# dpeerlab/segger

Hardware: AMD Instinct MI355X
Metric: edges scored/sec (tx->cell) fwd+bwd (higher is better)
Workload: dtype bf16; 1 GPU; C2: single Xenium-scale tile per GPU, 1000000 tx, 10000 nuclei, k=15 kNN (Ett=15000000, Etb=393796, Ep=2435646), training step fwd+bwd+Adam, attention dropout 0.2; parallelism=dp1

## Files before the change

### include/segger_amd.h

```cpp
#ifndef SEGGER_AMD_H
#define SEGGER_AMD_H

#include <stddef.h>
#include <stdint.h>

#ifdef __cplusplus
extern "C" {
#endif

#if defined(__GNUC__) || defined(__clang__)
#pragma GCC visibility push(default)
#endif

#define SEGGER_ABI_VERSION 30

enum segger_status {
  SEGGER_OK = 0,
  SEGGER_EINVAL = -1,
  SEGGER_EUNSUPPORTED = -2,
  SEGGER_EHIP = -3,
  SEGGER_EWORKSPACE = -4
};

enum segger_dtype { SEGGER_F32 = 0, SEGGER_BF16 = 1, SEGGER_F16 = 2 };

typedef void* segger_stream_t;

int segger_abi_version(void);
const char* segger_last_error(void);
// ... 381 lines not shown
                             float max_period, float* grad_w0, float* grad_b0, void* workspace, size_t workspace_bytes,
                             segger_stream_t stream);
int segger_posmlp_fwd(const float* pos, const int64_t* batch, const float* mins, const float* maxs, int64_t n, float eps,
                      float max_period, const void* w0, const float* b0, const void* w2, const float* b2, void* pe,
                      void* z1, float* pn, void* h1, void* pe_pre, int32_t gelu, int32_t dtype, segger_stream_t stream);
size_t segger_posmlp_bwd_workspace_bytes(int64_t n_rows);
int segger_posmlp_bwd(const void* g, int64_t ld_g, const void* z1, const float* pn, const void* w2_t, int64_t n_rows,
                      float max_period, int32_t dtype, float* grad_w0, float* grad_b0, float* grad_w2, float* grad_b2,
                      void* workspace, size_t workspace_bytes, segger_stream_t stream);
size_t segger_posmlp_bwd_pair_workspace_bytes(int64_t n_rows_a, int64_t n_rows_b);
int segger_posmlp_bwd_pair(const void* g_a, int64_t ld_ga, const void* z1_a, const float* pn_a, int64_t n_rows_a,
                           const void* g_b, int64_t ld_gb, const void* z1_b, const float* pn_b, int64_t n_rows_b,
                           const void* w2_t, float max_period, int32_t dtype, float* grad_w0, float* grad_b0,
                           float* grad_w2, float* grad_b2, void* workspace, size_t workspace_bytes,
                           segger_stream_t stream);
int segger_posmlp_wgrad(const void* dz1, int64_t ld_dz1, const float* pn, int64_t n_rows, float max_period,
                        int32_t dtype, float* grad_w0, float* grad_b0, void* workspace, size_t workspace_bytes,
                        segger_stream_t stream);
int segger_embed_gelu_fwd(const float* table, const int32_t* ids, const void* pe, int64_t ld_pe, int64_t n,
                          int32_t n_rows_table, int32_t D, void* out, int64_t ld_out, int32_t dtype,
                          segger_stream_t stream);
size_t segger_embed_gelu_bwd_workspace_bytes(int64_t n, int32_t n_rows_table, int32_t D);
int segger_embed_gelu_bwd(const void* gx0, int64_t ld_g, const float* table, const void* pe, int64_t ld_pe,
                          int64_t n, int32_t n_rows_table, int32_t D, void* gpe, int64_t ld_gpe, float* gtable,
                          const int64_t* gene_ptr, const int32_t* gene_rows, void* workspace, size_t workspace_bytes,
                          int32_t dtype, segger_stream_t stream);
typedef struct segger_front_join_args {
  const float* table; const int32_t* ids; int32_t n_rows_table; int32_t D; int32_t dtype; int32_t reserved_;
  const void* pe; int64_t ld_pe; int64_t n_tx, n_bd;
  const void* xb; int64_t ld_xb;
// ... 42 lines not shown
```

### segger_amd/_lib.py

```python
from __future__ import annotations

import ctypes as C
import os
from typing import Optional

import torch

_HERE = os.path.dirname(os.path.abspath(__file__))
LIB_PATH = os.environ.get("SEGGER_AMD_LIB") or os.path.join(_HERE, "libsegger_amd.so")
ABI_VERSION = 30

SEGGER_F32, SEGGER_BF16, SEGGER_F16 = 0, 1, 2
DTYPE_CODE = {torch.float32: SEGGER_F32, torch.bfloat16: SEGGER_BF16, torch.float16: SEGGER_F16}


class SeggerAmdError(RuntimeError):
    pass


c_i64p = C.c_void_p
vp = C.c_void_p


class Csr(C.Structure):
    _fields_ = [("indptr", vp), ("col", vp), ("eid", vp),
# ... 234 lines not shown
    "segger_gatv2_fwd_pair": (C.c_int, [vp, vp, vp]),
    "segger_gatv2_bwd_pair": (C.c_int, [vp, vp, vp]),
    "segger_pack_refresh": (C.c_int, [vp, C.c_int32, C.c_int32, vp]),
    "segger_dropout_bits_many": (C.c_int, [vp, C.c_int32, C.c_int32, C.c_float, vp, vp]),
    "segger_step_advance": (C.c_int, [vp, C.c_int64, vp, vp]),
    "segger_step_draws": (C.c_int, [C.POINTER(StepDrawsArgs), vp]),
    "segger_segment_minmax_ex": (C.c_int, [vp, vp, C.c_int64, C.c_int64, vp, vp, C.c_int32, vp]),
    "segger_triplet_partial_count": (C.c_int64, [C.c_int64]),
    "segger_loss_combine_partials_fwd": (C.c_int, [vp, vp, vp, vp, vp, C.c_int32, vp, vp]),
    "segger_posmlp_bwd_workspace_bytes": (C.c_size_t, [C.c_int64]),
    "segger_posmlp_bwd": (C.c_int, [vp, C.c_int64, vp, vp, vp, C.c_int64, C.c_float, C.c_int32, vp, vp, vp, vp, vp,
                                    C.c_size_t, vp]),
    "segger_posmlp_bwd_pair_workspace_bytes": (C.c_size_t, [C.c_int64, C.c_int64]),
    "segger_posmlp_bwd_pair": (C.c_int, [vp, C.c_int64, vp, vp, C.c_int64, vp, C.c_int64, vp, vp, C.c_int64, vp, C.c_float,
                                         C.c_int32, vp, vp, vp, vp, vp, C.c_size_t, vp]),
    "segger_linear_wgrad_dx_gate_supported": (C.c_int, [C.c_int32, C.c_int32, C.c_int32]),
    "segger_linear_wgrad_dx": (C.c_int, [vp, C.c_int64, vp, C.c_int64, vp, C.c_int64, C.c_int32, C.c_int32, C.c_int32, vp, vp,
                                         vp, C.c_int64, vp, C.c_int64, vp, C.c_size_t, vp]),
    "segger_posfreq": (C.c_int, [vp, vp, vp, vp, C.c_int64, C.c_int32, C.c_float, C.c_float, vp, C.c_int32, vp]),
    "segger_posenc_poly_supported": (C.c_int, [C.c_int32, C.c_int32]),
    "segger_posenc_poly_coef": (C.c_int, [vp, vp, C.c_int32, C.c_int32, C.c_float, vp, vp]),
    "segger_posenc_poly_fwd": (C.c_int, [vp, vp, vp, vp, C.c_int64, C.c_float, vp, C.c_int32, vp, vp, vp, vp]),
    "segger_posenc_poly_wgrad_workspace_bytes": (C.c_size_t, [C.c_int64, C.c_int32]),
    "segger_posenc_poly_wgrad": (C.c_int, [vp, C.c_int64, vp, C.c_int64, C.c_int32, C.c_int32, C.c_float, vp, vp, vp, C.c_size_t, vp]),
    "segger_embed_gelu_fwd": (C.c_int, [vp, vp, vp, C.c_int64, C.c_int64, C.c_int32, C.c_int32, vp, C.c_int64, C.c_int32, vp]),
    "segger_linear_fwd_f32_split_rowbias": (C.c_int, [vp, C.c_int64, vp, vp, C.c_int64, vp, vp, C.c_int64, C.c_int64, C.c_int32, C.c_int32, vp]),
    "segger_linear_fwd_f32_act": (C.c_int, [vp, C.c_int64, vp, vp, vp, C.c_int64, vp, C.c_int64, C.c_int32, C.c_int64, C.c_int32, C.c_int32, vp]),
    "segger_linear_fwd_f32_gate": (C.c_int, [vp, C.c_int64, vp, C.c_int32, vp, C.c_int64, C.c_int32, vp, C.c_int64, C.c_int64, C.c_int32, C.c_int32, vp]),
    "segger_f32_split_planes": (C.c_int, [vp, C.c_int32, C.c_int32, C.c_int32, vp, vp]),
    "segger_f32_split_planes_many": (C.c_int, [vp, C.c_int32, vp]),
# ... 97 lines not shown
```

### segger_amd/csrc/common.h

```cpp
#pragma once
#include <hip/hip_runtime.h>
#include <stdint.h>
#include <stdio.h>
#include <stdarg.h>
#include "../../include/segger_amd.h"

namespace segger {

void set_error(const char* fmt, ...);
int hip_fail(hipError_t e, const char* what);

#define SEGGER_REQUIRE(cond, ...)                 \
  do {                                            \
    if (!(cond)) {                                \
      ::segger::set_error(__VA_ARGS__);           \
      return SEGGER_EINVAL;                       \
    }                                             \
  } while (0)

#define SEGGER_HIP(call)                                        \
  do {                                                          \
    hipError_t _e = (call);                                     \
    if (_e != hipSuccess) return ::segger::hip_fail(_e, #call); \
  } while (0)
// ... 10 lines not shown
  static int cache[64] = {};
  int dev = 0;
  if (hipGetDevice(&dev) != hipSuccess || dev < 0) return 0;
  if (dev < 64 && cache[dev] > 0) return cache[dev];
  int n = 0;
  if (hipDeviceGetAttribute(&n, hipDeviceAttributeMultiprocessorCount, dev) != hipSuccess) n = 0;
  if (dev < 64 && n > 0) cache[dev] = n;
  return n;
}

int linear_f32_launch(const void* x, int64_t ldx, const void* w, const float* bias, void* y, int64_t ldy, int64_t n_rows,
                      int k_in, int m_out, hipStream_t stream, const float* rowbias = nullptr, const int32_t* rowidx = nullptr,
                      int64_t ld_rb = 0, const float* gate = nullptr, int64_t ld_gate = 0, int gate_kind = 0,
                      float* y_act = nullptr, int64_t ld_yact = 0, int act_kind = 0);
size_t wgrad_f32_workspace_bytes(int64_t n_rows, int m_out, int k_in);
bool wgrad_f32_split_shape_ok(int m, int k);
int64_t wgrad_f32_split_grid(int64_t n_rows, int m, int k);
int wgrad_f32_split_launch(const float* dy, int64_t ld_dy, const float* x, int64_t ld_x, int64_t n_rows, int m_out, int k_in,
                           float* partial, int64_t* n_slabs, hipStream_t stream);
int wgrad_f32_launch(const void* dy, int64_t ld_dy, const void* x, int64_t ld_x, int64_t n_rows, int m_out, int k_in,
                     float* partial, int64_t* n_slabs, hipStream_t stream);

struct ReduceSeg {
  const float* partial; int64_t n_slabs; int64_t width; int64_t split; float* out0; float* out1;
  float* scratch;
};
constexpr int kReduceGroups = 32;
bool defer_reduce(const ReduceSeg& seg, hipStream_t stream);

constexpr int kWave = 64;
// ... 170 lines not shown
```

### segger_amd/csrc/linear_wgrad.hip

```cpp
#include <cstdlib>
#include "common.h"

namespace segger {
namespace {

typedef __bf16   bf16x8 __attribute__((ext_vector_type(8)));
typedef _Float16 f16x8  __attribute__((ext_vector_type(8)));
typedef __bf16   bf16x2v __attribute__((ext_vector_type(2)));
typedef _Float16 f16x2v  __attribute__((ext_vector_type(2)));
typedef float    f32x16 __attribute__((ext_vector_type(16)));
typedef short    s16x4  __attribute__((ext_vector_type(4)));
typedef uint32_t u32x2  __attribute__((ext_vector_type(2)));
typedef uint32_t u32x4v __attribute__((ext_vector_type(4)));

constexpr int kStageRows = 16;

template <typename T> struct WgMfma;
template <> struct WgMfma<bf16_t> {
  static __device__ __forceinline__ f32x16 run(u32x4 a, u32x4 b, f32x16 c) {
    return __builtin_amdgcn_mfma_f32_32x32x16_bf16(__builtin_bit_cast(bf16x8, a), __builtin_bit_cast(bf16x8, b), c, 0, 0, 0);
  }
  static __device__ __forceinline__ f32x4 run16(u32x4 a, u32x4 b, f32x4 c) {
    return __builtin_amdgcn_mfma_f32_16x16x32_bf16(__builtin_bit_cast(bf16x8, a), __builtin_bit_cast(bf16x8, b), c, 0, 0, 0);
  }
// ... 338 lines not shown
  const void* z1;
  const float* pn;
  const void* w2t;
  int64_t n_rows, n_stages, stages_per_block;
  float* part2;
  float* part0;
  float log_max_period;
};
constexpr int kPbD = 64, kPbF = 256;
constexpr int kPbS = kPbD * 2 + 64;
constexpr int kPbTile = kStageRows * kPbS;
constexpr int kPbOffZ = kPbTile, kPbOffP = 2 * kPbTile;
constexpr int kPbBuf = 8 * 1024;
constexpr int kPbAhead = 6, kPbSlots = kPbAhead + 2;
constexpr int kPbWidth2 = kPbD * kPbD + kPbD, kPbWidth0 = kPbD * kPbF + kPbD;

__device__ __forceinline__ float sigmoid_fast(float z) {
  return __builtin_amdgcn_rcpf(1.0f + __builtin_amdgcn_exp2f(-1.4426950408889634f * z));
}

template <typename T>
__global__ __launch_bounds__(512, 2) void posmlp_bwd_kernel(PosBwdParams pa, PosBwdParams pb, int n_first) {
  const bool second = (int)blockIdx.x >= n_first;
  const PosBwdParams& p = second ? pb : pa;
  const int bid = second ? (int)blockIdx.x - n_first : (int)blockIdx.x;
  constexpr int D = kPbD, F = kPbF, S = kPbS, NW = 8, BUF = kPbBuf, NB = kPbSlots, TILE = kPbTile;
  __shared__ __attribute__((aligned(1024))) unsigned char lds[NB * BUF + 4 * TILE];
  unsigned char* tile_h = lds + NB * BUF;
  unsigned char* tile_d = tile_h + 2 * TILE;
  const int tid = threadIdx.x, lane = tid & 63;
  const int wave = __builtin_amdgcn_readfirstlane(tid >> 6);
  const T* __restrict__ gp = static_cast<const T*>(p.g);
  const T* __restrict__ zp = static_cast<const T*>(p.z1);

  const int64_t s_beg = (int64_t)bid * p.stages_per_block;
  int64_t s_end = s_beg + p.stages_per_block;
  if (s_end > p.n_stages) s_end = p.n_stages;
  const int n_local = (int)(s_end > s_beg ? s_end - s_beg : 0);
  const int64_t row_beg = s_beg * kStageRows;
  int64_t span_rows = p.n_rows > row_beg ? p.n_rows - row_beg : 0;
  if (span_rows > (int64_t)n_local * kStageRows) span_rows = (int64_t)n_local * kStageRows;
  i32x4 rs; int stage_bytes, voff;
// ... 20 lines not shown
  auto issue = [&](int local_stage) {
    lds_dma16(rs, lds_base + (uint32_t)((local_stage % NB) * BUF + wave * 1024), voff, local_stage * stage_bytes);
  };

  const int g4 = lane >> 4, i16 = lane & 15, tq = i16 >> 2, tp = i16 & 3;
  const int off_a = (8 * (g4 >> 1) + tq) * S + (16 * (g4 & 1) + 4 * tp) * 2;
  const int wm2 = wave & 1, wk2 = (wave >> 1) & 1;
  const int dq = lane >> 4, dj = lane & 15;
  const int r = lane & 31, h = lane >> 5;
  const bool lo_half = wave < 4;

  f32x16 acc2, acc0[2];
#pragma unroll
  for (int e = 0; e < 16; ++e) { acc2[e] = 0.f; acc0[0][e] = 0.f; acc0[1][e] = 0.f; }
  float db2 = 0.f, db0[2] = {0.f, 0.f};
  const float omega = expf(-p.log_max_period * (float)((32 * wave + r) % (F / 2)) / (float)(F / 2)) * 0.15915494309189535f;
  u32x4 wf[2] = {u32x4{0, 0, 0, 0}, u32x4{0, 0, 0, 0}};
  if (lo_half) {
    const T* wt = static_cast<const T*>(p.w2t);
#pragma unroll
    for (int ks = 0; ks < 2; ++ks)
      wf[ks] = *reinterpret_cast<const u32x4*>(wt + (16 * wave + dj) * D + 32 * ks + 8 * dq);
  }
  __builtin_amdgcn_s_waitcnt(0x0F70);
  asm volatile("" : "+v"(wf[0]), "+v"(wf[1]));

  auto consume = [&](int t) {
    const unsigned char* pb = lds + (t % NB) * BUF;
    const unsigned char* th = tile_h + (t & 1) * TILE;
    const unsigned char* td = tile_d + (t & 1) * TILE;
    if (lo_half) {
      const u32x2 lo = lds_read_tr(pb + off_a + wm2 * 64), hi = lds_read_tr(pb + off_a + wm2 * 64 + 4 * S);
      const u32x4 fa = u32x4{lo.x, lo.y, hi.x, hi.y};
      if (wk2 == 0) {
        db2 = WgMfma<T>::sum2(fa.x, db2); db2 = WgMfma<T>::sum2(fa.y, db2);
        db2 = WgMfma<T>::sum2(fa.z, db2); db2 = WgMfma<T>::sum2(fa.w, db2);
      }
      const u32x2 lo2 = lds_read_tr(th + off_a + wk2 * 64), hi2 = lds_read_tr(th + off_a + wk2 * 64 + 4 * S);
      acc2 = WgMfma<T>::run(fa, u32x4{lo2.x, lo2.y, hi2.x, hi2.y}, acc2);
    }
    u32x4 fd[2];
#pragma unroll
    for (int a = 0; a < 2; ++a) {
      const u32x2 lo = lds_read_tr(td + off_a + a * 64), hi = lds_read_tr(td + off_a + a * 64 + 4 * S);
      fd[a] = u32x4{lo.x, lo.y, hi.x, hi.y};
    }
    if (wave == 7) {
#pragma unroll
      for (int a = 0; a < 2; ++a) {
        float d = db0[a];
        d = WgMfma<T>::sum2(fd[a].x, d); d = WgMfma<T>::sum2(fd[a].y, d);
        d = WgMfma<T>::sum2(fd[a].z, d); d = WgMfma<T>::sum2(fd[a].w, d);
        db0[a] = d;
      }
    }
// ... 35 lines not shown
#pragma unroll
      for (int ks = 0; ks < 2; ++ks) {
        const u32x4 fy = *reinterpret_cast<const u32x4*>(base + dj * S + (32 * ks + 8 * dq) * 2);
        dacc = WgMfma<T>::run16(wf[ks], fy, dacc);
      }
      const u32x2 zv = *reinterpret_cast<const u32x2*>(base + kPbOffZ + dj * S + (16 * wave + 4 * dq) * 2);
      float z[4];
      Vec8<T>::unpack2(zv.x, z[0], z[1]);
      Vec8<T>::unpack2(zv.y, z[2], z[3]);
      float o[4] = {dacc.x, dacc.y, dacc.z, dacc.w};
#pragma unroll
      for (int e = 0; e < 4; ++e) {
        const float sg = sigmoid_fast(z[e]);
        o[e] *= sg * (1.0f + z[e] * (1.0f - sg));
      }
      *reinterpret_cast<u32x2*>(tile_d + (s & 1) * TILE + dj * S + (16 * wave + 4 * dq) * 2) =
          u32x2{Vec8<T>::pack(o[0], o[1]), Vec8<T>::pack(o[2], o[3])};
    }
    if (s > 0) consume(s - 1);
  }
  if (n_local > 0) {
    __builtin_amdgcn_s_waitcnt(0xC07F);
    __builtin_amdgcn_s_barrier();
    consume(n_local - 1);
  }
  __builtin_amdgcn_s_waitcnt(0x0F70);

  float* out2 = p.part2 + (int64_t)bid * kPbWidth2;
  float* out0 = p.part0 + (int64_t)bid * kPbWidth0;
#pragma unroll
  for (int e = 0; e < 16; ++e) {
    const int m = (e & 3) + 8 * (e >> 2) + 4 * h;
    if (lo_half) out2[(32 * wm2 + m) * D + 32 * wk2 + r] = acc2[e];
#pragma unroll
    for (int a = 0; a < 2; ++a) out0[(32 * a + m) * F + 32 * wave + r] = acc0[a][e];
  }
  if (lo_half && wk2 == 0) {
    const float d = db2 + __shfl_xor(db2, 32, 64);
    if (h == 0) out2[D * D + 32 * wm2 + r] = d;
  }
  if (wave == 7) {
#pragma unroll
    for (int a = 0; a < 2; ++a) {
      const float d = db0[a] + __shfl_xor(db0[a], 32, 64);
      if (h == 0) out0[D * F + 32 * a + r] = d;
    }
  }
}

constexpr int kRedGroups = 32;
__global__ __launch_bounds__(256) void wgrad_reduce1_kernel(const float* __restrict__ partial, int64_t n_slabs, int64_t width,
                                                           float* __restrict__ part2) {
  const int64_t e = (int64_t)blockIdx.x * 256 + threadIdx.x;
  if (e >= width) return;
  const int g = blockIdx.y;
  float s0 = 0.f, s1 = 0.f, s2 = 0.f, s3 = 0.f;
  int64_t s = g;
  for (; s + 3 * kRedGroups < n_slabs; s += 4 * kRedGroups) {
    s0 += partial[s * width + e];                    s1 += partial[(s + kRedGroups) * width + e];
    s2 += partial[(s + 2 * kRedGroups) * width + e]; s3 += partial[(s + 3 * kRedGroups) * width + e];
  }
  for (; s < n_slabs; s += kRedGroups) s0 += partial[s * width + e];
// ... 395 lines not shown

static int64_t posmlp_bwd_grid(int64_t n_rows) {
  const int64_t stages = (n_rows + kStageRows - 1) / kStageRows;
  const int64_t want = (stages + kMinStagesPerBlock - 1) / kMinStagesPerBlock;
  const int64_t cap = 2 * kNumCu;
  return want < cap ? (want < 1 ? 1 : want) : cap;
}

extern "C" size_t segger_posmlp_bwd_pair_workspace_bytes(int64_t n_rows_a, int64_t n_rows_b) {
  const int64_t grid = (n_rows_a > 0 ? posmlp_bwd_grid(n_rows_a) : 0) + (n_rows_b > 0 ? posmlp_bwd_grid(n_rows_b) : 0);
  if (grid == 0) return 16;
  return (size_t)(grid + kRedGroups) * (size_t)(kPbWidth2 + kPbWidth0) * sizeof(float);
}
extern "C" size_t segger_posmlp_bwd_workspace_bytes(int64_t n_rows) { return segger_posmlp_bwd_pair_workspace_bytes(n_rows, 0); }

extern "C" int segger_posmlp_bwd_pair(const void* g_a, int64_t ld_ga, const void* z1_a, const float* pn_a, int64_t n_rows_a,
                                      const void* g_b, int64_t ld_gb, const void* z1_b, const float* pn_b, int64_t n_rows_b,
                                      const void* w2_t, float max_period, int32_t dtype, float* grad_w0, float* grad_b0,
                                      float* grad_w2, float* grad_b2, void* workspace, size_t workspace_bytes,
                                      segger_stream_t stream_) {
  hipStream_t stream = (hipStream_t)stream_;
  SEGGER_REQUIRE(n_rows_a >= 0 && n_rows_b >= 0, "segger_posmlp_bwd: negative size");
  SEGGER_REQUIRE(dtype == SEGGER_BF16 || dtype == SEGGER_F16, "segger_posmlp_bwd: bf16 / f16 only");
  SEGGER_REQUIRE(grad_w0 && grad_b0 && grad_w2 && grad_b2, "segger_posmlp_bwd: NULL output");
  if (n_rows_a == 0 && n_rows_b == 0) {
    SEGGER_HIP(hipMemsetAsync(grad_w0, 0, (size_t)kPbD * kPbF * sizeof(float), stream));
    SEGGER_HIP(hipMemsetAsync(grad_b0, 0, (size_t)kPbD * sizeof(float), stream));
    SEGGER_HIP(hipMemsetAsync(grad_w2, 0, (size_t)kPbD * kPbD * sizeof(float), stream));
    SEGGER_HIP(hipMemsetAsync(grad_b2, 0, (size_t)kPbD * sizeof(float), stream));
    return SEGGER_OK;
  }
  SEGGER_REQUIRE(w2_t && aligned16(w2_t), "segger_posmlp_bwd: NULL / misaligned W2^T");
  const size_t need = segger_posmlp_bwd_pair_workspace_bytes(n_rows_a, n_rows_b);
  if (workspace == nullptr || workspace_bytes < need) {
    set_error("segger_posmlp_bwd: workspace %zu < %zu bytes", workspace_bytes, need);
    return SEGGER_EWORKSPACE;
  }
  const int64_t grid_a = n_rows_a > 0 ? posmlp_bwd_grid(n_rows_a) : 0, grid_b = n_rows_b > 0 ? posmlp_bwd_grid(n_rows_b) : 0;
  const int64_t grid = grid_a + grid_b;
  float* part2 = static_cast<float*>(workspace);
  float* part0 = part2 + (size_t)(grid + kRedGroups) * kPbWidth2;
  const float lmp = logf(max_period);
  auto side = [&](const void* g, int64_t ld_g, const void* z1, const float* pn, int64_t n_rows, int64_t grid_s, int64_t first,
                  PosBwdParams& out) -> int {
    if (n_rows == 0) { out = PosBwdParams{nullptr, kPbD, nullptr, nullptr, w2_t, 0, 0, 0, part2, part0, lmp}; return SEGGER_OK; }
    SEGGER_REQUIRE(g && z1 && pn, "segger_posmlp_bwd: NULL input");
    SEGGER_REQUIRE(aligned16(g) && aligned16(z1) && aligned16(pn) && ld_g >= kPbD && (ld_g * 2) % 16 == 0,
                   "segger_posmlp_bwd: rows must be 16-byte aligned");
    const int64_t stages = (n_rows + kStageRows - 1) / kStageRows;
    SEGGER_REQUIRE(((stages + grid_s - 1) / grid_s + kPbAhead) * kStageRows * ld_g * 2 < (int64_t)kOutOfRange,
                   "segger_posmlp_bwd: a workgroup's row slab exceeds 1 GiB");
    out = PosBwdParams{g, ld_g, z1, pn, w2_t, n_rows, stages, (stages + grid_s - 1) / grid_s, part2 + (size_t)first * kPbWidth2,
                       part0 + (size_t)first * kPbWidth0, lmp};
    return SEGGER_OK;
  };
  PosBwdParams pa, pb;
  int rc = side(g_a, ld_ga, z1_a, pn_a, n_rows_a, grid_a, 0, pa);
  if (rc != SEGGER_OK) return rc;
  rc = side(g_b, ld_gb, z1_b, pn_b, n_rows_b, grid_b, grid_a, pb);
  if (rc != SEGGER_OK) return rc;
  if (dtype == SEGGER_BF16)
    hipLaunchKernelGGL((posmlp_bwd_kernel<bf16_t>), dim3((unsigned)grid), dim3(512), 0, stream, pa, pb, (int)grid_a);
  else
    hipLaunchKernelGGL((posmlp_bwd_kernel<f16_t>), dim3((unsigned)grid), dim3(512), 0, stream, pa, pb, (int)grid_a);
  SEGGER_LAUNCH_CHECK("posmlp_bwd_kernel");
  rc = reduce_partials(part2, grid, kPbD, kPbD, grad_w2, grad_b2, stream);
  if (rc != SEGGER_OK) return rc;
  return reduce_partials(part0, grid, kPbD, kPbF, grad_w0, grad_b0, stream);
}

extern "C" int segger_posmlp_bwd(const void* g, int64_t ld_g, const void* z1, const float* pn, const void* w2_t,
                                 int64_t n_rows, float max_period, int32_t dtype, float* grad_w0, float* grad_b0,
                                 float* grad_w2, float* grad_b2, void* workspace, size_t workspace_bytes,
                                 segger_stream_t stream_) {
  return segger_posmlp_bwd_pair(g, ld_g, z1, pn, n_rows, nullptr, kPbD, nullptr, nullptr, 0, w2_t, max_period, dtype, grad_w0,
                                grad_b0, grad_w2, grad_b2, workspace, workspace_bytes, stream_);
}
```

### segger_amd/csrc/posenc_poly.hip

```cpp
#include "common.h"

namespace segger {
namespace {

constexpr int kTerms = 13;
constexpr int kCoefStride = 16;
constexpr int kMaxBlocks = 1024;

__device__ __forceinline__ double feature_freq(int j, int half, float log_max_period) {
  return (double)expf(-log_max_period * (float)j / (float)half);
}

__device__ __constant__ double kInvFact[kTerms] = {1.0, 1.0, 1.0 / 2, 1.0 / 6, 1.0 / 24, 1.0 / 120, 1.0 / 720, 1.0 / 5040, 1.0 / 40320,
                                                  1.0 / 362880, 1.0 / 3628800, 1.0 / 39916800, 1.0 / 479001600};

__global__ __launch_bounds__(256) void poly_coef_kernel(const float* __restrict__ w0, const float* __restrict__ b0, int fd,
                                                        float log_max_period, float* __restrict__ coef) {
  __shared__ double red[16][kCoefStride];
  const int m = blockIdx.x, d = threadIdx.x % kCoefStride, part = threadIdx.x / kCoefStride, half = fd / 2;
  double s = 0.0;
  if (d < kTerms) {
    const float* row = w0 + (int64_t)m * fd + ((d & 1) ? half : 0);
    for (int j = part; j < half; j += 16) {
      const double om = feature_freq(j, half, log_max_period);
// ... 148 lines not shown
      pw *= om2;
    }
    grad_w0[(int64_t)m * fd + f] = (float)s;
  }
  if (grad_b0 && threadIdx.x == 0) grad_b0[m] = (float)mom[0];
}

int64_t poly_grid(int64_t rows, int dim) {
  const int64_t rows_per_block = 4 * (64 / (dim / 4));
  int64_t blocks = (rows + rows_per_block * 8 - 1) / (rows_per_block * 8);
  if (blocks > kMaxBlocks) blocks = kMaxBlocks;
  return blocks < 1 ? 1 : blocks;
}

}
}

using namespace segger;

extern "C" int segger_posenc_poly_supported(int32_t freq_dim, int32_t dim) {
  return (dim == 32 || dim == 64 || dim == 128) && freq_dim >= 2 && freq_dim % 2 == 0 && freq_dim <= 4096;
}

extern "C" int segger_posenc_poly_coef(const float* w0, const float* b0, int32_t freq_dim, int32_t dim, float max_period,
                                       float* coef, segger_stream_t stream) {
  SEGGER_REQUIRE(segger_posenc_poly_supported(freq_dim, dim), "segger_posenc_poly_coef: dim 32 / 64 / 128, even freq_dim <= 4096");
  SEGGER_REQUIRE(w0 && coef && max_period > 1.f, "segger_posenc_poly_coef: NULL pointer or max_period <= 1");
  hipLaunchKernelGGL(poly_coef_kernel, dim3((unsigned)dim), dim3(256), 0, (hipStream_t)stream, w0, b0, (int)freq_dim,
                     logf(max_period), coef);
  SEGGER_LAUNCH_CHECK("poly_coef_kernel");
// ... 34 lines not shown
    if (grad_b0) SEGGER_HIP(hipMemsetAsync(grad_b0, 0, (size_t)dim * sizeof(float), (hipStream_t)stream));
    return SEGGER_OK;
  }
  SEGGER_REQUIRE(dz1 && pn && aligned16(dz1) && ld >= dim && ld % 4 == 0, "segger_posenc_poly_wgrad: dz1 NULL, misaligned or ld < dim");
  const size_t need = segger_posenc_poly_wgrad_workspace_bytes(n_rows, dim);
  if (!workspace || workspace_bytes < need) {
    set_error("segger_posenc_poly_wgrad: workspace %zu < %zu bytes", workspace_bytes, need);
    return SEGGER_EWORKSPACE;
  }
  const int64_t blocks = poly_grid(n_rows, dim);
  PolyMoments p{dz1, ld, pn, n_rows, static_cast<float*>(workspace)};
  if (dim == 32) hipLaunchKernelGGL((poly_moments_kernel<32>), dim3((unsigned)blocks), dim3(256), 0, (hipStream_t)stream, p);
  else if (dim == 64) hipLaunchKernelGGL((poly_moments_kernel<64>), dim3((unsigned)blocks), dim3(256), 0, (hipStream_t)stream, p);
  else hipLaunchKernelGGL((poly_moments_kernel<128>), dim3((unsigned)blocks), dim3(256), 0, (hipStream_t)stream, p);
  SEGGER_LAUNCH_CHECK("poly_moments_kernel");
  hipLaunchKernelGGL(poly_wgrad_finish_kernel, dim3((unsigned)dim), dim3(256), 0, (hipStream_t)stream,
                     static_cast<const float*>(workspace), (int)blocks, (int)dim, (int)freq_dim, logf(max_period), grad_w0, grad_b0);
  SEGGER_LAUNCH_CHECK("poly_wgrad_finish_kernel");
  return SEGGER_OK;
}
```

### segger_amd/ops.py

```python
from __future__ import annotations

import ctypes as C
from typing import Optional, Tuple

import torch
from torch import Tensor

from . import _lib
from ._lib import DTYPE_CODE
from . import graph as _graph
from .graph import EdgeCSR, EdgeGraph


def _rows(t: Tensor, width: int, name: str) -> Tuple[int, int]:
    sh = t.shape
    if len(sh) != 2 or sh[1] != width:
        raise ValueError(f"{name}: expected [n, {width}], got {tuple(sh)}")
    st = t.stride()
    if sh[0] > 1:
        if st[1] != 1:
            raise ValueError(f"{name}: last dimension must be contiguous")
        return t.data_ptr(), st[0]
    return t.data_ptr(), max(width, st[0])

# ... 2011 lines not shown
        batch = batch.to(device=dev, dtype=torch.int64).contiguous()
    out = torch.empty((n, 2, freq_dim), dtype=dtype, device=dev)
    with _lib.on_device(dev):
        rc = lib.segger_posfreq(pos.data_ptr(), _lib.ptr(batch), mins.data_ptr(), maxs.data_ptr(), n, freq_dim,
                                eps, max_period, out.data_ptr(), DTYPE_CODE[dtype], _lib.stream_ptr(dev))
    _lib.check(rc, "segger_posfreq")
    return out


def posmlp_supported(freq_dim: int, dim: int, dtype: torch.dtype) -> bool:
    return dtype in (torch.bfloat16, torch.float16) and bool(
        _lib.load().segger_posmlp_supported(int(freq_dim), int(dim), DTYPE_CODE[dtype]))


FUSED_POSMLP_BWD = True


class _PosMlp(torch.autograd.Function):

    @staticmethod
    def forward(ctx, pos, batch, mins, maxs, eps, max_period, dtype, train, gelu, w0, b0, w2, b2):
        _lib.require_cuda(pos, w0)
        lib = _lib.load()
        dev = pos.device
        pos = pos.to(torch.float32).contiguous()
        n = int(pos.shape[0])
        if batch is not None:
            batch = batch.to(device=dev, dtype=torch.int64).contiguous()
        pk0 = _pack_for((w0,), (b0,)).get(dtype, dev)
        pk2 = _pack_for((w2,), (b2,)).get(dtype, dev)
# ... 33 lines not shown
            gpe = torch.ops.aten.gelu_backward(gpe.to(dt), pre)
        g = gpe.to(dt).reshape(-1, d)
        if g.shape[0] > 1 and g.stride(1) != 1:
            g = g.contiguous()
        if ctx.pk2.key != ctx.key2:
            raise RuntimeError("the positional MLP's weights changed between this forward and its backward")
        need = ctx.needs_input_grad
        if h1 is None:
            lib = _lib.load()
            dev = z1.device
            gw0 = torch.empty((d, 4 * d), dtype=torch.float32, device=dev)
            gb0 = torch.empty(d, dtype=torch.float32, device=dev)
            gw2 = torch.empty((d, d), dtype=torch.float32, device=dev)
            gb2 = torch.empty(d, dtype=torch.float32, device=dev)
            n_rows = int(g.shape[0])
            ws_bytes = lib.segger_posmlp_bwd_workspace_bytes(n_rows)
            ws = torch.empty(ws_bytes, dtype=torch.uint8, device=dev)
            gp, ldg = _rows(g, d, "g")
            with _lib.on_device(dev):
                rc = lib.segger_posmlp_bwd(gp, ldg, z1.data_ptr(), pn.data_ptr(), ctx.pk2.wt.data_ptr(), n_rows,
                                           ctx.max_period, DTYPE_CODE[dt], gw0.data_ptr(), gb0.data_ptr(), gw2.data_ptr(),
                                           gb2.data_ptr(), ws.data_ptr(), ws_bytes, _lib.stream_ptr(dev))
            _lib.check(rc, "segger_posmlp_bwd")
            _defer_keep(ws, gw0, gb0, gw2, gb2)
            return (None, None, None, None, None, None, None, None, None, gw0 if need[9] else None,
                    gb0 if need[10] else None, gw2 if need[11] else None, gb2 if need[12] else None)
        gw2, gb2 = linear_wgrad_launch(g, h1)
        lib0 = _lib.load()
        dz1 = torch.empty_like(z1)
        wt = ctx.pk2.wt
        gp, ldg = _rows(g, d, "g")
        with _lib.on_device(z1.device):
            rc = lib0.segger_linear_fwd_silu_grad(gp, ldg, wt.data_ptr(), z1.data_ptr(), d, dz1.data_ptr(), d,
                                                  int(g.shape[0]), d, d, DTYPE_CODE[dt], _lib.stream_ptr(z1.device))
        _lib.check(rc, "segger_linear_fwd_silu_grad")
        lib = _lib.load()
        dev = z1.device
        gw0 = torch.empty((d, 4 * d), dtype=torch.float32, device=dev)
# ... 58 lines not shown

        def rows(g):
            if g is None:
                return None, d, 0
            g = g.to(dt).reshape(-1, d)
            if g.shape[0] > 1 and g.stride(1) != 1:
                g = g.contiguous()
            gp, ldg = _rows(g, d, "g")
            return (g, gp), ldg, int(g.shape[0])
        ga, lda, na = rows(gpre_a)
        gb, ldb, nb = rows(gpe_b)
        gw0 = torch.empty((d, 4 * d), dtype=torch.float32, device=dev)
        gb0 = torch.empty(d, dtype=torch.float32, device=dev)
        gw2 = torch.empty((d, d), dtype=torch.float32, device=dev)
        gb2 = torch.empty(d, dtype=torch.float32, device=dev)
        ws_bytes = lib.segger_posmlp_bwd_pair_workspace_bytes(na, nb)
        ws = torch.empty(ws_bytes, dtype=torch.uint8, device=dev)
        with _lib.on_device(dev):
            rc = lib.segger_posmlp_bwd_pair(ga[1] if ga else None, lda, z1_a.data_ptr(), pn_a.data_ptr(), na,
                                            gb[1] if gb else None, ldb, z1_b.data_ptr(), pn_b.data_ptr(), nb,
                                            ctx.pk2.wt.data_ptr(), ctx.max_period, DTYPE_CODE[dt], gw0.data_ptr(), gb0.data_ptr(),
                                            gw2.data_ptr(), gb2.data_ptr(), ws.data_ptr(), ws_bytes, _lib.stream_ptr(dev))
        _lib.check(rc, "segger_posmlp_bwd_pair")
        _defer_keep(ws, gw0, gb0, gw2, gb2, ga, gb)
        need = ctx.needs_input_grad
        return (None,) * 11 + (gw0 if need[11] else None, gb0 if need[12] else None, gw2 if need[13] else None,
                               gb2 if need[14] else None)


def posmlp_pair_supported(w0: Tensor, b0, w2: Tensor, b2, dtype: torch.dtype) -> bool:
    return (FUSED_POSMLP_BWD and b0 is not None and b2 is not None and posmlp_supported(w0.shape[1], w0.shape[0], dtype)
            and tuple(w2.shape) == (w0.shape[0], w0.shape[0]) and torch.is_grad_enabled()
            and any(t.requires_grad for t in (w0, b0, w2, b2)))


def posmlp_pair(pos_a: Tensor, batch_a, mins_a: Tensor, maxs_a: Tensor, pos_b: Tensor, batch_b, mins_b: Tensor, maxs_b: Tensor,
                w0: Tensor, b0: Tensor, w2: Tensor, b2: Tensor, dtype: torch.dtype, eps: float = 1e-8, max_period: float = 10000.0):
    if not posmlp_pair_supported(w0, b0, w2, b2, dtype):
# ... 458 lines not shown
```

Measured before the change: 60.91 million edges/s.

## Compute positional-MLP first-layer weight gradient via polynomial moments in fused backward

Adds a moments variant of the fused positional-MLP backward kernel. Instead of running an MFMA of dz1 against the sinusoidal frequency features and writing wide per-block W0 partials, it accumulates 13 power moments of the normalized position per output column. The existing poly_wgrad_finish kernel then expands these moments into grad_w0 and grad_b0. This is meant to cut matrix work, LDS use and partial-buffer traffic in the backward pass, at the cost of relying on a truncated polynomial expansion of the sin/cos features, which may change gradient accuracy.

```diff
diff --git a/include/segger_amd.h b/include/segger_amd.h
--- a/include/segger_amd.h
+++ b/include/segger_amd.h
@@ -12,7 +12,7 @@
 #pragma GCC visibility push(default)
 #endif
 
-#define SEGGER_ABI_VERSION 30
+#define SEGGER_ABI_VERSION 31
 
 enum segger_status {
   SEGGER_OK = 0,
@@ -424,6 +424,12 @@
                            const void* w2_t, float max_period, int32_t dtype, float* grad_w0, float* grad_b0,
                            float* grad_w2, float* grad_b2, void* workspace, size_t workspace_bytes,
                            segger_stream_t stream);
+size_t segger_posmlp_bwd_pair_moments_workspace_bytes(int64_t n_rows_a, int64_t n_rows_b);
+int segger_posmlp_bwd_pair_moments(const void* g_a, int64_t ld_ga, const void* z1_a, const float* pn_a, int64_t n_rows_a,
+                                   const void* g_b, int64_t ld_gb, const void* z1_b, const float* pn_b, int64_t n_rows_b,
+                                   const void* w2_t, float max_period, int32_t dtype, float* grad_w0, float* grad_b0,
+                                   float* grad_w2, float* grad_b2, void* workspace, size_t workspace_bytes,
+                                   segger_stream_t stream);
 int segger_posmlp_wgrad(const void* dz1, int64_t ld_dz1, const float* pn, int64_t n_rows, float max_period,
                         int32_t dtype, float* grad_w0, float* grad_b0, void* workspace, size_t workspace_bytes,
                         segger_stream_t stream);
diff --git a/segger_amd/_lib.py b/segger_amd/_lib.py
--- a/segger_amd/_lib.py
+++ b/segger_amd/_lib.py
@@ -8,7 +8,7 @@
 
 _HERE = os.path.dirname(os.path.abspath(__file__))
 LIB_PATH = os.environ.get("SEGGER_AMD_LIB") or os.path.join(_HERE, "libsegger_amd.so")
-ABI_VERSION = 30
+ABI_VERSION = 31
 
 SEGGER_F32, SEGGER_BF16, SEGGER_F16 = 0, 1, 2
 DTYPE_CODE = {torch.float32: SEGGER_F32, torch.bfloat16: SEGGER_BF16, torch.float16: SEGGER_F16}
@@ -273,6 +273,9 @@
     "segger_posmlp_bwd_pair_workspace_bytes": (C.c_size_t, [C.c_int64, C.c_int64]),
     "segger_posmlp_bwd_pair": (C.c_int, [vp, C.c_int64, vp, vp, C.c_int64, vp, C.c_int64, vp, vp, C.c_int64, vp, C.c_float,
                                          C.c_int32, vp, vp, vp, vp, vp, C.c_size_t, vp]),
+    "segger_posmlp_bwd_pair_moments_workspace_bytes": (C.c_size_t, [C.c_int64, C.c_int64]),
+    "segger_posmlp_bwd_pair_moments": (C.c_int, [vp, C.c_int64, vp, vp, C.c_int64, vp, C.c_int64, vp, vp, C.c_int64, vp,
+                                                 C.c_float, C.c_int32, vp, vp, vp, vp, vp, C.c_size_t, vp]),
     "segger_linear_wgrad_dx_gate_supported": (C.c_int, [C.c_int32, C.c_int32, C.c_int32]),
     "segger_linear_wgrad_dx": (C.c_int, [vp, C.c_int64, vp, C.c_int64, vp, C.c_int64, C.c_int32, C.c_int32, C.c_int32, vp, vp,
                                          vp, C.c_int64, vp, C.c_int64, vp, C.c_size_t, vp]),
diff --git a/segger_amd/csrc/common.h b/segger_amd/csrc/common.h
--- a/segger_amd/csrc/common.h
+++ b/segger_amd/csrc/common.h
@@ -48,6 +48,8 @@
                       int64_t ld_rb = 0, const float* gate = nullptr, int64_t ld_gate = 0, int gate_kind = 0,
                       float* y_act = nullptr, int64_t ld_yact = 0, int act_kind = 0);
 size_t wgrad_f32_workspace_bytes(int64_t n_rows, int m_out, int k_in);
+int poly_wgrad_finish(const float* part, int64_t nblocks, int dim, int fd, float log_max_period, float* grad_w0,
+                      float* grad_b0, hipStream_t stream);
 bool wgrad_f32_split_shape_ok(int m, int k);
 int64_t wgrad_f32_split_grid(int64_t n_rows, int m, int k);
 int wgrad_f32_split_launch(const float* dy, int64_t ld_dy, const float* x, int64_t ld_x, int64_t n_rows, int m_out, int k_in,
diff --git a/segger_amd/csrc/linear_wgrad.hip b/segger_amd/csrc/linear_wgrad.hip
--- a/segger_amd/csrc/linear_wgrad.hip
+++ b/segger_amd/csrc/linear_wgrad.hip
@@ -376,18 +376,21 @@
 constexpr int kPbBuf = 8 * 1024;
 constexpr int kPbAhead = 6, kPbSlots = kPbAhead + 2;
 constexpr int kPbWidth2 = kPbD * kPbD + kPbD, kPbWidth0 = kPbD * kPbF + kPbD;
+constexpr int kPbTerms = 13, kPbMomStride = 16;
+constexpr int kPbWidthM = kPbD * kPbMomStride;
 
 __device__ __forceinline__ float sigmoid_fast(float z) {
   return __builtin_amdgcn_rcpf(1.0f + __builtin_amdgcn_exp2f(-1.4426950408889634f * z));
 }
 
-template <typename T>
-__global__ __launch_bounds__(512, 2) void posmlp_bwd_kernel(PosBwdParams pa, PosBwdParams pb, int n_first) {
+constexpr int posmlp_bwd_lds_bytes(bool mom) { return kPbSlots * kPbBuf + (mom ? 2 : 4) * kPbTile; }
+template <typename T, bool MOM>
+__device__ __forceinline__ void posmlp_bwd_body(const PosBwdParams& pa, const PosBwdParams& pb, int n_first,
+                                                unsigned char* lds) {
   const bool second = (int)blockIdx.x >= n_first;
   const PosBwdParams& p = second ? pb : pa;
   const int bid = second ? (int)blockIdx.x - n_first : (int)blockIdx.x;
   constexpr int D = kPbD, F = kPbF, S = kPbS, NW = 8, BUF = kPbBuf, NB = kPbSlots, TILE = kPbTile;
-  __shared__ __attribute__((aligned(1024))) unsigned char lds[NB * BUF + 4 * TILE];
   unsigned char* tile_h = lds + NB * BUF;
   unsigned char* tile_d = tile_h + 2 * TILE;
   const int tid = threadIdx.x, lane = tid & 63;
@@ -438,6 +441,12 @@
 #pragma unroll
   for (int e = 0; e < 16; ++e) { acc2[e] = 0.f; acc0[0][e] = 0.f; acc0[1][e] = 0.f; }
   float db2 = 0.f, db0[2] = {0.f, 0.f};
+  float mom[4][kPbTerms];
+#pragma unroll
+  for (int e = 0; e < 4; ++e) {
+#pragma unroll
+    for (int d = 0; d < kPbTerms; ++d) mom[e][d] = 0.f;
+  }
   const float omega = expf(-p.log_max_period * (float)((32 * wave + r) % (F / 2)) / (float)(F / 2)) * 0.15915494309189535f;
   u32x4 wf[2] = {u32x4{0, 0, 0, 0}, u32x4{0, 0, 0, 0}};
   if (lo_half) {
@@ -463,6 +472,7 @@
       const u32x2 lo2 = lds_read_tr(th + off_a + wk2 * 64), hi2 = lds_read_tr(th + off_a + wk2 * 64 + 4 * S);
       acc2 = WgMfma<T>::run(fa, u32x4{lo2.x, lo2.y, hi2.x, hi2.y}, acc2);
     }
+    if constexpr (MOM) return;
     u32x4 fd[2];
 #pragma unroll
     for (int a = 0; a < 2; ++a) {
@@ -528,8 +538,19 @@
         const float sg = sigmoid_fast(z[e]);
         o[e] *= sg * (1.0f + z[e] * (1.0f - sg));
       }
-      *reinterpret_cast<u32x2*>(tile_d + (s & 1) * TILE + dj * S + (16 * wave + 4 * dq) * 2) =
-          u32x2{Vec8<T>::pack(o[0], o[1]), Vec8<T>::pack(o[2], o[3])};
+      if constexpr (MOM) {
+        const float x = reinterpret_cast<const float*>(base + kPbOffP)[dj];
+        float pw = 1.0f;
+#pragma unroll
+        for (int d = 0; d < kPbTerms; ++d) {
+#pragma unroll
+          for (int e = 0; e < 4; ++e) mom[e][d] = fmaf(o[e], pw, mom[e][d]);
+          pw *= x;
+        }
+      } else {
+        *reinterpret_cast<u32x2*>(tile_d + (s & 1) * TILE + dj * S + (16 * wave + 4 * dq) * 2) =
+            u32x2{Vec8<T>::pack(o[0], o[1]), Vec8<T>::pack(o[2], o[3])};
+      }
     }
     if (s > 0) consume(s - 1);
   }
@@ -541,25 +562,53 @@
   __builtin_amdgcn_s_waitcnt(0x0F70);
 
   float* out2 = p.part2 + (int64_t)bid * kPbWidth2;
-  float* out0 = p.part0 + (int64_t)bid * kPbWidth0;
+  float* out0 = p.part0 + (int64_t)bid * (MOM ? kPbWidthM : kPbWidth0);
 #pragma unroll
   for (int e = 0; e < 16; ++e) {
     const int m = (e & 3) + 8 * (e >> 2) + 4 * h;
     if (lo_half) out2[(32 * wm2 + m) * D + 32 * wk2 + r] = acc2[e];
-#pragma unroll
-    for (int a = 0; a < 2; ++a) out0[(32 * a + m) * F + 32 * wave + r] = acc0[a][e];
+    if constexpr (!MOM) {
+#pragma unroll
+      for (int a = 0; a < 2; ++a) out0[(32 * a + m) * F + 32 * wave + r] = acc0[a][e];
+    }
   }
   if (lo_half && wk2 == 0) {
     const float d = db2 + __shfl_xor(db2, 32, 64);
     if (h == 0) out2[D * D + 32 * wm2 + r] = d;
   }
-  if (wave == 7) {
+  if constexpr (MOM) {
+    if (lo_half) {
+#pragma unroll
+      for (int e = 0; e < 4; ++e) {
+        float* col = out0 + (16 * wave + 4 * dq + e) * kPbMomStride;
+#pragma unroll
+        for (int d = 0; d < kPbTerms; ++d) {
+          float a = mom[e][d];
+          a += __shfl_xor(a, 1, 64); a += __shfl_xor(a, 2, 64);
+          a += __shfl_xor(a, 4, 64); a += __shfl_xor(a, 8, 64);
+          if (dj == 0) col[d] = a;
+        }
+        if (dj < kPbMomStride - kPbTerms) col[kPbTerms + dj] = 0.f;
+      }
+    }
+  } else if (wave == 7) {
 #pragma unroll
     for (int a = 0; a < 2; ++a) {
       const float d = db0[a] + __shfl_xor(db0[a], 32, 64);
       if (h == 0) out0[D * F + 32 * a + r] = d;
     }
   }
+}
+
+template <typename T>
+__global__ __launch_bounds__(512, 2) void posmlp_bwd_kernel(PosBwdParams pa, PosBwdParams pb, int n_first) {
+  __shared__ __attribute__((aligned(1024))) unsigned char lds[posmlp_bwd_lds_bytes(false)];
+  posmlp_bwd_body<T, false>(pa, pb, n_first, lds);
+}
+template <typename T>
+__global__ __launch_bounds__(512, 2) void posmlp_bwd_moments_kernel(PosBwdParams pa, PosBwdParams pb, int n_first) {
+  __shared__ __attribute__((aligned(1024))) unsigned char lds[posmlp_bwd_lds_bytes(true)];
+  posmlp_bwd_body<T, true>(pa, pb, n_first, lds);
 }
 
 constexpr int kRedGroups = 32;
@@ -985,11 +1034,17 @@
 }
 extern "C" size_t segger_posmlp_bwd_workspace_bytes(int64_t n_rows) { return segger_posmlp_bwd_pair_workspace_bytes(n_rows, 0); }
 
-extern "C" int segger_posmlp_bwd_pair(const void* g_a, int64_t ld_ga, const void* z1_a, const float* pn_a, int64_t n_rows_a,
-                                      const void* g_b, int64_t ld_gb, const void* z1_b, const float* pn_b, int64_t n_rows_b,
-                                      const void* w2_t, float max_period, int32_t dtype, float* grad_w0, float* grad_b0,
-                                      float* grad_w2, float* grad_b2, void* workspace, size_t workspace_bytes,
-                                      segger_stream_t stream_) {
+extern "C" size_t segger_posmlp_bwd_pair_moments_workspace_bytes(int64_t n_rows_a, int64_t n_rows_b) {
+  const int64_t grid = (n_rows_a > 0 ? posmlp_bwd_grid(n_rows_a) : 0) + (n_rows_b > 0 ? posmlp_bwd_grid(n_rows_b) : 0);
+  if (grid == 0) return 16;
+  return ((size_t)(grid + kRedGroups) * kPbWidth2 + (size_t)grid * kPbWidthM) * sizeof(float);
+}
+
+static int posmlp_bwd_pair_launch(bool moments, const void* g_a, int64_t ld_ga, const void* z1_a, const float* pn_a,
+                                  int64_t n_rows_a, const void* g_b, int64_t ld_gb, const void* z1_b, const float* pn_b,
+                                  int64_t n_rows_b, const void* w2_t, float max_period, int32_t dtype, float* grad_w0,
+                                  float* grad_b0, float* grad_w2, float* grad_b2, void* workspace, size_t workspace_bytes,
+                                  segger_stream_t stream_) {
   hipStream_t stream = (hipStream_t)stream_;
   SEGGER_REQUIRE(n_rows_a >= 0 && n_rows_b >= 0, "segger_posmlp_bwd: negative size");
   SEGGER_REQUIRE(dtype == SEGGER_BF16 || dtype == SEGGER_F16, "segger_posmlp_bwd: bf16 / f16 only");
@@ -1002,7 +1057,8 @@
     return SEGGER_OK;
   }
   SEGGER_REQUIRE(w2_t && aligned16(w2_t), "segger_posmlp_bwd: NULL / misaligned W2^T");
-  const size_t need = segger_posmlp_bwd_pair_workspace_bytes(n_rows_a, n_rows_b);
+  const size_t need = moments ? segger_posmlp_bwd_pair_moments_workspace_bytes(n_rows_a, n_rows_b)
+                              : segger_posmlp_bwd_pair_workspace_bytes(n_rows_a, n_rows_b);
   if (workspace == nullptr || workspace_bytes < need) {
     set_error("segger_posmlp_bwd: workspace %zu < %zu bytes", workspace_bytes, need);
     return SEGGER_EWORKSPACE;
@@ -1011,6 +1067,7 @@
   const int64_t grid = grid_a + grid_b;
   float* part2 = static_cast<float*>(workspace);
   float* part0 = part2 + (size_t)(grid + kRedGroups) * kPbWidth2;
+  const int64_t width0 = moments ? kPbWidthM : kPbWidth0;
   const float lmp = logf(max_period);
   auto side = [&](const void* g, int64_t ld_g, const void* z1, const float* pn, int64_t n_rows, int64_t grid_s, int64_t first,
                   PosBwdParams& out) -> int {
@@ -1022,7 +1079,7 @@
     SEGGER_REQUIRE(((stages + grid_s - 1) / grid_s + kPbAhead) * kStageRows * ld_g * 2 < (int64_t)kOutOfRange,
                    "segger_posmlp_bwd: a workgroup's row slab exceeds 1 GiB");
     out = PosBwdParams{g, ld_g, z1, pn, w2_t, n_rows, stages, (stages + grid_s - 1) / grid_s, part2 + (size_t)first * kPbWidth2,
-                       part0 + (size_t)first * kPbWidth0, lmp};
+                       part0 + (size_t)first * width0, lmp};
     return SEGGER_OK;
   };
   PosBwdParams pa, pb;
@@ -1030,14 +1087,33 @@
   if (rc != SEGGER_OK) return rc;
   rc = side(g_b, ld_gb, z1_b, pn_b, n_rows_b, grid_b, grid_a, pb);
   if (rc != SEGGER_OK) return rc;
-  if (dtype == SEGGER_BF16)
-    hipLaunchKernelGGL((posmlp_bwd_kernel<bf16_t>), dim3((unsigned)grid), dim3(512), 0, stream, pa, pb, (int)grid_a);
-  else
-    hipLaunchKernelGGL((posmlp_bwd_kernel<f16_t>), dim3((unsigned)grid), dim3(512), 0, stream, pa, pb, (int)grid_a);
-  SEGGER_LAUNCH_CHECK("posmlp_bwd_kernel");
+#define GO(K, T) hipLaunchKernelGGL((K<T>), dim3((unsigned)grid), dim3(512), 0, stream, pa, pb, (int)grid_a)
+  if (dtype == SEGGER_BF16) { if (moments) GO(posmlp_bwd_moments_kernel, bf16_t); else GO(posmlp_bwd_kernel, bf16_t); }
+  else { if (moments) GO(posmlp_bwd_moments_kernel, f16_t); else GO(posmlp_bwd_kernel, f16_t); }
+#undef GO
+  SEGGER_LAUNCH_CHECK(moments ? "posmlp_bwd_moments_kernel" : "posmlp_bwd_kernel");
   rc = reduce_partials(part2, grid, kPbD, kPbD, grad_w2, grad_b2, stream);
   if (rc != SEGGER_OK) return rc;
+  if (moments) return poly_wgrad_finish(part0, grid, kPbD, kPbF, lmp, grad_w0, grad_b0, stream);
   return reduce_partials(part0, grid, kPbD, kPbF, grad_w0, grad_b0, stream);
+}
+
+extern "C" int segger_posmlp_bwd_pair(const void* g_a, int64_t ld_ga, const void* z1_a, const float* pn_a, int64_t n_rows_a,
+                                      const void* g_b, int64_t ld_gb, const void* z1_b, const float* pn_b, int64_t n_rows_b,
+                                      const void* w2_t, float max_period, int32_t dtype, float* grad_w0, float* grad_b0,
+                                      float* grad_w2, float* grad_b2, void* workspace, size_t workspace_bytes,
+                                      segger_stream_t stream) {
+  return posmlp_bwd_pair_launch(false, g_a, ld_ga, z1_a, pn_a, n_rows_a, g_b, ld_gb, z1_b, pn_b, n_rows_b, w2_t, max_period,
+                                dtype, grad_w0, grad_b0, grad_w2, grad_b2, workspace, workspace_bytes, stream);
+}
+
+extern "C" int segger_posmlp_bwd_pair_moments(const void* g_a, int64_t ld_ga, const void* z1_a, const float* pn_a,
+                                              int64_t n_rows_a, const void* g_b, int64_t ld_gb, const void* z1_b,
+                                              const float* pn_b, int64_t n_rows_b, const void* w2_t, float max_period,
+                                              int32_t dtype, float* grad_w0, float* grad_b0, float* grad_w2, float* grad_b2,
+                                              void* workspace, size_t workspace_bytes, segger_stream_t stream) {
+  return posmlp_bwd_pair_launch(true, g_a, ld_ga, z1_a, pn_a, n_rows_a, g_b, ld_gb, z1_b, pn_b, n_rows_b, w2_t, max_period,
+                                dtype, grad_w0, grad_b0, grad_w2, grad_b2, workspace, workspace_bytes, stream);
 }
 
 extern "C" int segger_posmlp_bwd(const void* g, int64_t ld_g, const void* z1, const float* pn, const void* w2_t,
diff --git a/segger_amd/csrc/posenc_poly.hip b/segger_amd/csrc/posenc_poly.hip
--- a/segger_amd/csrc/posenc_poly.hip
+++ b/segger_amd/csrc/posenc_poly.hip
@@ -186,6 +186,15 @@
 }
 
 }
+
+int poly_wgrad_finish(const float* part, int64_t nblocks, int dim, int fd, float log_max_period, float* grad_w0,
+                      float* grad_b0, hipStream_t stream) {
+  hipLaunchKernelGGL(poly_wgrad_finish_kernel, dim3((unsigned)dim), dim3(256), 0, stream, part, (int)nblocks, dim, fd,
+                     log_max_period, grad_w0, grad_b0);
+  SEGGER_LAUNCH_CHECK("poly_wgrad_finish_kernel");
+  return SEGGER_OK;
+}
+
 }
 
 using namespace segger;
@@ -250,8 +259,6 @@
   else if (dim == 64) hipLaunchKernelGGL((poly_moments_kernel<64>), dim3((unsigned)blocks), dim3(256), 0, (hipStream_t)stream, p);
   else hipLaunchKernelGGL((poly_moments_kernel<128>), dim3((unsigned)blocks), dim3(256), 0, (hipStream_t)stream, p);
   SEGGER_LAUNCH_CHECK("poly_moments_kernel");
-  hipLaunchKernelGGL(poly_wgrad_finish_kernel, dim3((unsigned)dim), dim3(256), 0, (hipStream_t)stream,
-                     static_cast<const float*>(workspace), (int)blocks, (int)dim, (int)freq_dim, logf(max_period), grad_w0, grad_b0);
-  SEGGER_LAUNCH_CHECK("poly_wgrad_finish_kernel");
-  return SEGGER_OK;
-}
+  return poly_wgrad_finish(static_cast<const float*>(workspace), blocks, (int)dim, (int)freq_dim, logf(max_period), grad_w0,
+                           grad_b0, (hipStream_t)stream);
+}
diff --git a/segger_amd/ops.py b/segger_amd/ops.py
--- a/segger_amd/ops.py
+++ b/segger_amd/ops.py
@@ -2049,6 +2049,7 @@
 
 
 FUSED_POSMLP_BWD = True
+MOMENT_POSMLP_BWD = True
 
 
 class _PosMlp(torch.autograd.Function):
@@ -2112,14 +2113,24 @@
             gw2 = torch.empty((d, d), dtype=torch.float32, device=dev)
             gb2 = torch.empty(d, dtype=torch.float32, device=dev)
             n_rows = int(g.shape[0])
-            ws_bytes = lib.segger_posmlp_bwd_workspace_bytes(n_rows)
-            ws = torch.empty(ws_bytes, dtype=torch.uint8, device=dev)
             gp, ldg = _rows(g, d, "g")
-            with _lib.on_device(dev):
-                rc = lib.segger_posmlp_bwd(gp, ldg, z1.data_ptr(), pn.data_ptr(), ctx.pk2.wt.data_ptr(), n_rows,
-                                           ctx.max_period, DTYPE_CODE[dt], gw0.data_ptr(), gb0.data_ptr(), gw2.data_ptr(),
-                                           gb2.data_ptr(), ws.data_ptr(), ws_bytes, _lib.stream_ptr(dev))
-            _lib.check(rc, "segger_posmlp_bwd")
+            if MOMENT_POSMLP_BWD:
+                ws_bytes = lib.segger_posmlp_bwd_pair_moments_workspace_bytes(n_rows, 0)
+                ws = torch.empty(ws_bytes, dtype=torch.uint8, device=dev)
+                with _lib.on_device(dev):
+                    rc = lib.segger_posmlp_bwd_pair_moments(gp, ldg, z1.data_ptr(), pn.data_ptr(), n_rows, None, d, None,
+                                                            None, 0, ctx.pk2.wt.data_ptr(), ctx.max_period, DTYPE_CODE[dt],
+                                                            gw0.data_ptr(), gb0.data_ptr(), gw2.data_ptr(), gb2.data_ptr(),
+                                                            ws.data_ptr(), ws_bytes, _lib.stream_ptr(dev))
+                _lib.check(rc, "segger_posmlp_bwd_pair_moments")
+            else:
+                ws_bytes = lib.segger_posmlp_bwd_workspace_bytes(n_rows)
+                ws = torch.empty(ws_bytes, dtype=torch.uint8, device=dev)
+                with _lib.on_device(dev):
+                    rc = lib.segger_posmlp_bwd(gp, ldg, z1.data_ptr(), pn.data_ptr(), ctx.pk2.wt.data_ptr(), n_rows,
+                                               ctx.max_period, DTYPE_CODE[dt], gw0.data_ptr(), gb0.data_ptr(), gw2.data_ptr(),
+                                               gb2.data_ptr(), ws.data_ptr(), ws_bytes, _lib.stream_ptr(dev))
+                _lib.check(rc, "segger_posmlp_bwd")
             _defer_keep(ws, gw0, gb0, gw2, gb2)
             return (None, None, None, None, None, None, None, None, None, gw0 if need[9] else None,
                     gb0 if need[10] else None, gw2 if need[11] else None, gb2 if need[12] else None)
@@ -2208,14 +2219,15 @@
         gb0 = torch.empty(d, dtype=torch.float32, device=dev)
         gw2 = torch.empty((d, d), dtype=torch.float32, device=dev)
         gb2 = torch.empty(d, dtype=torch.float32, device=dev)
-        ws_bytes = lib.segger_posmlp_bwd_pair_workspace_bytes(na, nb)
+        name = "segger_posmlp_bwd_pair_moments" if MOMENT_POSMLP_BWD else "segger_posmlp_bwd_pair"
+        ws_bytes = getattr(lib, name + "_workspace_bytes")(na, nb)
         ws = torch.empty(ws_bytes, dtype=torch.uint8, device=dev)
         with _lib.on_device(dev):
-            rc = lib.segger_posmlp_bwd_pair(ga[1] if ga else None, lda, z1_a.data_ptr(), pn_a.data_ptr(), na,
-                                            gb[1] if gb else None, ldb, z1_b.data_ptr(), pn_b.data_ptr(), nb,
-                                            ctx.pk2.wt.data_ptr(), ctx.max_period, DTYPE_CODE[dt], gw0.data_ptr(), gb0.data_ptr(),
-                                            gw2.data_ptr(), gb2.data_ptr(), ws.data_ptr(), ws_bytes, _lib.stream_ptr(dev))
-        _lib.check(rc, "segger_posmlp_bwd_pair")
+            rc = getattr(lib, name)(ga[1] if ga else None, lda, z1_a.data_ptr(), pn_a.data_ptr(), na,
+                                    gb[1] if gb else None, ldb, z1_b.data_ptr(), pn_b.data_ptr(), nb,
+                                    ctx.pk2.wt.data_ptr(), ctx.max_period, DTYPE_CODE[dt], gw0.data_ptr(), gb0.data_ptr(),
+                                    gw2.data_ptr(), gb2.data_ptr(), ws.data_ptr(), ws_bytes, _lib.stream_ptr(dev))
+        _lib.check(rc, name)
         _defer_keep(ws, gw0, gb0, gw2, gb2, ga, gb)
         need = ctx.needs_input_grad
         return (None,) * 11 + (gw0 if need[11] else None, gb0 if need[12] else None, gw2 if need[13] else None,
```

Measured after the change: 61.16 million edges/s (median of 6 runs). No clear change (+0.4%).
